# jingjing12110/X-GGM

Hardware: AMD Instinct MI355X
Metric: train samples/sec (36-obj VQA batch); one step = plain + GGM pass, each fwd+bwd+clip+BertAdam (higher is better)
Workload: dtype bf16; 1 GPU; 1xMI355X bf16: VQA-CP-v2-shaped synthetic batch=32/GPU, 36 objects x 2048, 20 tokens, A=2274, LXMERT 9/5/5 + GCNx2, full fwd+bwd+clip+BertAdam x2 passes (plain pass first, KL x 8), dropout on, delta=5 branch mix; global_batch=32, parallelism=dp1, order=vqa, world_size=1, zero1=False, hip_graph=True

## Files before the change

include/xggm.h:

```cpp
#ifndef XGGM_H
#define XGGM_H

#include <stddef.h>
#include <stdint.h>

#ifdef __cplusplus
extern "C" {
#endif

typedef struct ihipStream_t* xggm_stream_t;

#define XGGM_VERSION 100

#define XGGM_ACT_NONE 0
#define XGGM_ACT_GELU 1
#define XGGM_ACT_SIGMOID 2
#define XGGM_ACT_TANH 3
#define XGGM_ACT_GELU_GRAD 4

#define XGGM_AGG_PLAIN 0
#define XGGM_AGG_TRANSPOSE 1
#define XGGM_AGG_SYMMETRIZE 2

int xggm_version(void);
const char* xggm_last_error(void);
typedef struct xggm_prefetch { const void* ptr[4]; size_t bytes[4]; int n; } xggm_prefetch;

int xggm_gemm_f32(const void* A, const void* B, void* C, int M, int N, int K, int64_t a_rs, int64_t a_ks, int64_t b_ns,
                  int64_t b_ks, int64_t ldc, int batch, int64_t a_bs, int64_t b_bs, int64_t c_bs, const float* bias,
                  const void* residual, void* preact, const void* aux, float* colsum, int act, int c_f32, int accumulate,
                  float alpha, xggm_stream_t stream);
int xggm_gemm_bf16(const void* A, const void* B, void* C, int M, int N, int K, int64_t a_rs, int64_t a_ks, int64_t b_ns,
                   int64_t b_ks, int64_t ldc, int batch, int64_t a_bs, int64_t b_bs, int64_t c_bs, const float* bias,
                   const void* residual, void* preact, const void* aux, float* colsum, int act, int c_f32, int accumulate,
                   float alpha, xggm_stream_t stream);
typedef struct xggm_gemm_problem {
    const void* A;
    const void* B;
    void* C;
    int M, N, K;
    int64_t a_rs, a_ks, b_ns, b_ks, ldc;
    int batch;
    int64_t a_bs, b_bs, c_bs;
    const float* bias;
    const void* residual;
    void* preact;
    const void* aux;
    float* colsum;
    int act, c_f32, accumulate;
    float alpha;
    float* sqsum;
    const float* scale_a;
    const float* scale_b;
    void* c8;
    const float* c8_qscale;
    float* c8_amax;
    int amax_slots;
} xggm_gemm_problem;
int xggm_gemm_grouped_f32(const xggm_gemm_problem* probs, int n, int tile, xggm_stream_t stream);
int xggm_gemm_grouped_bf16(const xggm_gemm_problem* probs, int n, int tile, xggm_stream_t stream);
int xggm_gemm_fp8e4m3(const void* A, const void* B, void* C, int M, int N, int K, int64_t a_rs, int64_t b_ns, int64_t ldc,
                      const float* scale_a, const float* scale_b, const float* bias, const void* residual, void* preact,
                      int act, int c_f32, xggm_stream_t stream);
int xggm_gemm_grouped_fp8e4m3(const xggm_gemm_problem* probs, int n, int tile, xggm_stream_t stream);
int xggm_fp8_scale_update(float* amax, float* hist, float* qscale, float* dscale, int64_t* pos, int n, int hist_len,
                          float margin, int shrink, int bump, int amax_slots, xggm_stream_t stream);
int xggm_quantize_fp8e4m3_f32(const void* x, void* y, int64_t n, const float* qscale, float* amax, xggm_stream_t stream);
int xggm_quantize_fp8e4m3_bf16(const void* x, void* y, int64_t n, const float* qscale, float* amax, xggm_stream_t stream);
int xggm_gemm_set_group_tile(int v);
int xggm_gemm_set_generic(int on);
int xggm_gemm_set_tile(int variant);
int xggm_colsum_f32(const void* x, float* out, int M, int N, int64_t ld, float* ws, size_t ws_bytes,
                    xggm_stream_t stream);
int xggm_colsum_bf16(const void* x, float* out, int M, int N, int64_t ld, float* ws, size_t ws_bytes,
                     xggm_stream_t stream);
size_t xggm_colsum_workspace_bytes(int M, int N);

int xggm_attn_fwd_f32(const void* q, const void* k, const void* v, const float* mask, void* out, int B, int heads, int Sq,
                      int Sk, int head_dim, int64_t q_rs, int64_t k_rs, int64_t v_rs, int64_t o_rs, float scale, float p,
                      const uint64_t* rng, uint32_t sid, xggm_stream_t stream);
int xggm_attn_fwd_bf16(const void* q, const void* k, const void* v, const float* mask, void* out, int B, int heads, int Sq,
                       int Sk, int head_dim, int64_t q_rs, int64_t k_rs, int64_t v_rs, int64_t o_rs, float scale, float p,
                       const uint64_t* rng, uint32_t sid, xggm_stream_t stream);
int xggm_attn_bwd_f32(const void* q, const void* k, const void* v, const float* mask, const void* d_out, void* dq, void* dk,
                      void* dv, int B, int heads, int Sq, int Sk, int head_dim, int64_t q_rs, int64_t k_rs, int64_t v_rs,
                      int64_t o_rs, int64_t dq_rs, int64_t dk_rs, int64_t dv_rs, float scale, float p, const uint64_t* rng,
                      uint32_t sid, float* dbq, float* dbk, float* dbv, int64_t db_bs, xggm_stream_t stream);
int xggm_attn_bwd_bf16(const void* q, const void* k, const void* v, const float* mask, const void* d_out, void* dq,
                       void* dk, void* dv, int B, int heads, int Sq, int Sk, int head_dim, int64_t q_rs, int64_t k_rs,
                       int64_t v_rs, int64_t o_rs, int64_t dq_rs, int64_t dk_rs, int64_t dv_rs, float scale, float p,
                       const uint64_t* rng, uint32_t sid, float* dbq, float* dbk, float* dbv, int64_t db_bs,
                       xggm_stream_t stream);

typedef struct xggm_attn_problem {
    const void* q;
    const void* k;
    const void* v;
    const float* mask;
    void* out;
    int B, heads, Sq, Sk;
    int64_t q_rs, k_rs, v_rs, o_rs;
    float scale, p;
    uint32_t sid;
    const void* d_out;
    void* dq;
    void* dk;
    void* dv;
    int64_t dq_rs, dk_rs, dv_rs;
    float* dbq;
    float* dbk;
    float* dbv;
    int64_t db_bs;
    void* out8;
    const float* qscale;
    float* amax;
    int amax_slots;
} xggm_attn_problem;
int xggm_attn_fwd_grouped_f32(const xggm_attn_problem* probs, int n, int head_dim, const uint64_t* rng,
                              const xggm_prefetch* prefetch, xggm_stream_t stream);
int xggm_attn_fwd_grouped_bf16(const xggm_attn_problem* probs, int n, int head_dim, const uint64_t* rng,
                               const xggm_prefetch* prefetch, xggm_stream_t stream);
int xggm_attn_bwd_grouped_f32(const xggm_attn_problem* probs, int n, int head_dim, const uint64_t* rng,
                              const xggm_prefetch* prefetch, xggm_stream_t stream);
int xggm_attn_bwd_grouped_bf16(const xggm_attn_problem* probs, int n, int head_dim, const uint64_t* rng,
                               const xggm_prefetch* prefetch, xggm_stream_t stream);

int xggm_attn_set_scalar(int on);

int xggm_ln_fwd_f32(const void* in, const float* bias, const void* residual, const float* gamma, const float* beta,
                    void* out, void* z_out, float* stats, int M, int H, float eps, float p_pre, float p_post,
                    const uint64_t* rng, uint32_t sid_pre, uint32_t sid_post, int accumulate, float out_scale,
                    xggm_stream_t stream);
int xggm_ln_fwd_bf16(const void* in, const float* bias, const void* residual, const float* gamma, const float* beta,
                     void* out, void* z_out, float* stats, int M, int H, float eps, float p_pre, float p_post,
                     const uint64_t* rng, uint32_t sid_pre, uint32_t sid_post, int accumulate, float out_scale,
                     xggm_stream_t stream);
int xggm_ln_bwd_f32(const void* dy, const void* z, const float* stats, const float* gamma, void* d_in, void* d_res,
                    float* dgamma, float* dbeta, float* dbias, int M, int H, float p_pre, float p_post, const uint64_t* rng,
                    uint32_t sid_pre, uint32_t sid_post, float out_scale, int accumulate_dres, const void* gelu_aux,
                    float* ws, size_t ws_bytes, xggm_stream_t stream);
int xggm_ln_bwd_bf16(const void* dy, const void* z, const float* stats, const float* gamma, void* d_in, void* d_res,
                     float* dgamma, float* dbeta, float* dbias, int M, int H, float p_pre, float p_post,
                     const uint64_t* rng, uint32_t sid_pre, uint32_t sid_post, float out_scale, int accumulate_dres,
                     const void* gelu_aux, float* ws, size_t ws_bytes, xggm_stream_t stream);
typedef struct xggm_ln_fwd_problem {
    const void* in;
    const float* bias;
    const void* residual;
    const float* gamma;
    const float* beta;
    void* out;
    void* z_out;
    float* stats;
    int M;
    uint32_t sid_pre, sid_post;
    int in_slabs;
    void* out8;
    const float* qscale;
    float* amax;
    int amax_slots;
} xggm_ln_fwd_problem;
typedef struct xggm_ln_bwd_problem {
    const void* dy;
    const void* z;
    const float* stats;
    const float* gamma;
    void* d_in;
    void* d_res;
    float* dgamma;
    float* dbeta;
    float* dbias;
    const void* gelu_aux;
    float* ws;
    size_t ws_bytes;
    int M;
    uint32_t sid_pre, sid_post;
    int accumulate_dres;
} xggm_ln_bwd_problem;
int xggm_ln_fwd_grouped_f32(const xggm_ln_fwd_problem* probs, int n, int H, float eps, float p_pre, float p_post,
                            const uint64_t* rng, int accumulate, float out_scale, const xggm_prefetch* prefetch,
                            xggm_stream_t stream);
int xggm_ln_fwd_grouped_bf16(const xggm_ln_fwd_problem* probs, int n, int H, float eps, float p_pre, float p_post,
                             const uint64_t* rng, int accumulate, float out_scale, const xggm_prefetch* prefetch,
                             xggm_stream_t stream);
int xggm_ln_bwd_grouped_f32(const xggm_ln_bwd_problem* probs, int n, int H, float p_pre, float p_post,
                            const uint64_t* rng, float out_scale, const xggm_prefetch* prefetch, xggm_stream_t stream);
int xggm_ln_bwd_grouped_bf16(const xggm_ln_bwd_problem* probs, int n, int H, float p_pre, float p_post,
                             const uint64_t* rng, float out_scale, const xggm_prefetch* prefetch, xggm_stream_t stream);
typedef struct xggm_ln_sum_args {
    const void* in[4];
    const float* gamma[4];
    const float* beta[4];
    float* stats[4];
    uint32_t sid_post[4];
    void* out;
    int n, M, H;
    float eps, p_post;
    const uint64_t* rng;
} xggm_ln_sum_args;
int xggm_ln_sum_fwd_f32(const xggm_ln_sum_args* args, xggm_stream_t stream);
int xggm_ln_sum_fwd_bf16(const xggm_ln_sum_args* args, xggm_stream_t stream);
size_t xggm_ln_bwd_workspace_bytes(int M, int H);
size_t xggm_visn_embed_bwd_workspace_bytes(int M, int H);
typedef struct xggm_reduce_job {
    const float* ws;
    int nblk, K, H;
    float* target[3];
} xggm_reduce_job;
int xggm_partial_reduce_batch(const xggm_reduce_job* jobs, int n, xggm_stream_t stream);
int xggm_embed_fwd_f32(const int64_t* ids, const int64_t* seg, const void* word, const void* pos, const void* type,
                       const float* gamma, const float* beta, void* out, void* z_out, float* stats, int M, int Tlen, int H,
                       float eps, float p, const uint64_t* rng, uint32_t sid, void* out8, const float* qscale, float* amax,
                       int amax_slots, xggm_stream_t stream);
int xggm_embed_fwd_bf16(const int64_t* ids, const int64_t* seg, const void* word, const void* pos, const void* type,
                        const float* gamma, const float* beta, void* out, void* z_out, float* stats, int M, int Tlen, int H,
                        float eps, float p, const uint64_t* rng, uint32_t sid, void* out8, const float* qscale, float* amax,
                        int amax_slots, xggm_stream_t stream);
#define XGGM_SIDE_MAX 3
#define XGGM_SIDE_ADDITIVE_MASK 1
#define XGGM_SIDE_CAST_BF16 2
typedef struct xggm_side_jobs {
    int n;
    struct {
// ... 266 lines not shown
```

x-ggm_amd/csrc/gemm.hip:

```cpp
#include "common.h"
#include "xggm.h"

namespace {

typedef __attribute__((ext_vector_type(8))) short short8_t;
typedef __attribute__((ext_vector_type(4))) float float4_t;

struct GemmArgs {
    const void* A = nullptr;
    const void* B = nullptr;
    void* C = nullptr;
    int M = 0, N = 0, K = 0;
    int64_t a_rs = 0, a_ks = 0, b_ns = 0, b_ks = 0, ldc = 0;
    int64_t a_bs = 0, b_bs = 0, c_bs = 0;
    const float* bias = nullptr;
    const void* residual = nullptr;
    void* preact = nullptr;
    const void* aux = nullptr;
    float* colsum = nullptr;
    float* sqsum = nullptr;
    unsigned char* c8 = nullptr;
    const float* c8_qscale = nullptr;
    float* c8_amax = nullptr;
    int amax_slots = 1;
    const float* scale_a = nullptr;
    const float* scale_b = nullptr;
    int act = 0;
    int c_f32 = 0;
    int accumulate = 0;
    float alpha = 1.f;
    int a_mode = 0, b_mode = 0;
    int a_tail = 0, b_tail = 0;
    int a_rows = 0, b_rows = 0;
    int xcd_swizzle = 1;
    int batch = 1;
    int use_glds = 1;
    struct TileMap {
        int gx, gy, gxy;
        int xr, xc, rh, rw;
        int ncg, wb_last;
        unsigned m_rw, m_wbl, m_gxy;
    } tm = {};
#ifdef XGGM_STAMP
    long long* stamp = nullptr;
    int ablate = 0;
#endif
};

#ifdef XGGM_STAMP
long long* g_stamp = nullptr;
int g_ablate = 0;
#define ABLATE(g, bit) ((g).ablate & (bit))
#ifdef XGGM_KABLATE
#define KABLATE(g, bit) ((g).ablate & (bit))
#else
#define KABLATE(g, bit) false
#endif
#define STAMP(g, slot)                                                                                \
    do {                                                                                              \
        if ((g).stamp && threadIdx.x == 0)                                                            \
            (g).stamp[(int64_t)(blockIdx.x + gridDim.x * (blockIdx.y + gridDim.y * blockIdx.z)) * 8 + (slot)] = \
                __builtin_readcyclecounter();                                                         \
    } while (0)
#define SET_STAMP(g) ((g).stamp = g_stamp, (g).ablate = g_ablate)
#define STAMP_HW(g)                                                                                   \
    do {                                                                                              \
        if ((g).stamp && threadIdx.x == 0) {                                                          \
            unsigned hw, xcc;                                                                         \
            asm volatile("s_getreg_b32 %0, hwreg(HW_REG_HW_ID)" : "=s"(hw));                          \
            asm volatile("s_getreg_b32 %0, hwreg(HW_REG_XCC_ID)" : "=s"(xcc));                        \
            long long* q = (g).stamp + (int64_t)(blockIdx.x + gridDim.x * (blockIdx.y + gridDim.y * blockIdx.z)) * 8; \
            q[5] = hw;                                                                                \
            q[6] = xcc;                                                                               \
        }                                                                                             \
    } while (0)
#define XGGM_TRACE_BASE (8 * 8192)
__shared__ long long xg_trace[128];
#define TRACE(g, slot)                                                                                \
    do {                                                                                              \
        if (((g).ablate & 0x10000) && threadIdx.x == 0 && (slot) < 128) xg_trace[(slot)] = __builtin_readcyclecounter(); \
    } while (0)
#define TRACE_FLUSH(g)                                                                                \
    do {                                                                                              \
        if (((g).ablate & 0x10000) && threadIdx.x < 64) {                                                          \
            long long* q = (g).stamp + XGGM_TRACE_BASE +                                              \
                           (int64_t)(blockIdx.x + gridDim.x * (blockIdx.y + gridDim.y * blockIdx.z)) * 128; \
            q[threadIdx.x] = xg_trace[threadIdx.x];                                                   \
            q[threadIdx.x + 64] = xg_trace[threadIdx.x + 64];                                         \
        }                                                                                             \
    } while (0)
#else
#define TRACE(g, slot)
#define TRACE_FLUSH(g)
#define STAMP_HW(g)
#define ABLATE(g, bit) false
#define KABLATE(g, bit) false
#define STAMP(g, slot)
#define SET_STAMP(g)
#endif

template <typename T> struct Tile;
template <> struct Tile<bf16> {
    static constexpr int BK = 64;
    static constexpr int VEC = 8;
    static constexpr int LDK = BK + 8;
};
template <> struct Tile<float> {
    static constexpr int BK = 32;
    static constexpr int VEC = 4;
    static constexpr int LDK = BK + 4;
};

constexpr int BM = 64, BN = 64, NT = 256;
struct GemmHooks {
    bool force_generic = false;
    int tile_override = 0;
    int xcd_swizzle = 1;
    int glds_stages = 0;
    int single_grouped = 1;
    int no_8w = 0;
    int glds = 1;
    int group_tile = 0;
};
GemmHooks g_hooks;

template <typename T>
__device__ __forceinline__ void stage_tile(T* __restrict__ lds, const T* __restrict__ base, int64_t rs, int64_t ks, int r0,
                                           int k0, int R, int K, int mode, int tid) {
    constexpr int BK = Tile<T>::BK, VEC = Tile<T>::VEC, LDK = Tile<T>::LDK;
    typedef typename std::conditional<sizeof(T) == 2, short8_t, float4_t>::type vec_t;
    if (mode == 1) {
        constexpr int CPR = BK / VEC;
#pragma unroll
        for (int c = tid; c < 64 * CPR; c += NT) {
            const int row = c / CPR, kc = (c % CPR) * VEC;
            const int gr = r0 + row, gk = k0 + kc;
            vec_t v = {};
            if (gr < R && gk < K) v = *reinterpret_cast<const vec_t*>(base + (int64_t)gr * rs + gk);
            *reinterpret_cast<vec_t*>(lds + row * LDK + kc) = v;
        }
    } else if (mode == 2) {
        constexpr int CPL = 64 / VEC;
#pragma unroll
        for (int c = tid; c < BK * CPL; c += NT) {
            const int kl = c / CPL, rc = (c % CPL) * VEC;
            const int gr = r0 + rc, gk = k0 + kl;
            vec_t v = {};
            if (gr < R && gk < K) v = *reinterpret_cast<const vec_t*>(base + (int64_t)gk * ks + gr);
            const T* e = reinterpret_cast<const T*>(&v);
#pragma unroll
            for (int i = 0; i < VEC; ++i) lds[(rc + i) * LDK + kl] = e[i];
        }
    } else {
        for (int c = tid; c < 64 * BK; c += NT) {
            const int row = c / BK, kk = c % BK;
            const int gr = r0 + row, gk = k0 + kk;
            T v = from_f32<T>(0.0f);
            if (gr < R && gk < K) v = base[(int64_t)gr * rs + (int64_t)gk * ks];
            lds[row * LDK + kk] = v;
        }
    }
}

template <typename T> __device__ __forceinline__ float act_apply(int act, float v, float aux) {
    switch (act) {
        case XGGM_ACT_GELU: return gelu_f(v);
        case XGGM_ACT_SIGMOID: return sigmoid_f(v);
        case XGGM_ACT_TANH: return tanhf(v);
        case XGGM_ACT_GELU_GRAD: return v * gelu_grad_f(aux);
        default: return v;
    }
}

template <typename T>
__device__ __forceinline__ float epilogue_tile(const GemmArgs& g, const float4_t& acc, int row0, int col, int bz) {
    if (col >= g.N) return 0.f;
    const int64_t coff = (int64_t)bz * g.c_bs;
    const float bias = g.bias ? g.bias[col] : 0.0f;
    float csum = 0.f;
#pragma unroll
    for (int r = 0; r < 4; ++r) {
        const int row = row0 + r;
        if (row >= g.M) continue;
        const int64_t idx = coff + (int64_t)row * g.ldc + col;
        float v = g.alpha * acc[r] + bias;
        if (g.preact) reinterpret_cast<T*>(g.preact)[idx] = from_f32<T>(v);
        float aux = 0.0f;
        if (g.act == XGGM_ACT_GELU_GRAD) aux = to_f32(reinterpret_cast<const T*>(g.aux)[idx]);
        if (g.act != XGGM_ACT_NONE) {
            if (g.preact) v = round_to<T>(v);
            v = act_apply<T>(g.act, v, aux);
        }
        if (g.residual) v += to_f32(reinterpret_cast<const T*>(g.residual)[idx]);
        if (g.c_f32) {
            float* c = reinterpret_cast<float*>(g.C) + idx;
            *c = g.accumulate ? (*c + v) : v;
        } else {
            T* c = reinterpret_cast<T*>(g.C) + idx;
            *c = from_f32<T>(g.accumulate ? (to_f32(*c) + v) : v);
        }
        csum += v;
    }
    return csum;
}

template <typename T> __global__ __launch_bounds__(NT) void gemm_kernel(GemmArgs g) {
    constexpr int BK = Tile<T>::BK, LDK = Tile<T>::LDK;
    __shared__ __attribute__((aligned(16))) T As[BM * LDK];
    __shared__ __attribute__((aligned(16))) T Bs[BN * LDK];

    const int tid = threadIdx.x, lane = tid & 63, wid = tid >> 6;
    const int wm = (wid >> 1) * 32, wn = (wid & 1) * 32;
    const int m0 = blockIdx.y * BM, n0 = blockIdx.x * BN, bz = blockIdx.z;
    const T* A = reinterpret_cast<const T*>(g.A) + (int64_t)bz * g.a_bs;
    const T* B = reinterpret_cast<const T*>(g.B) + (int64_t)bz * g.b_bs;

    float4_t acc[2][2];
#pragma unroll
    for (int i = 0; i < 2; ++i)
#pragma unroll
        for (int j = 0; j < 2; ++j) acc[i][j] = (float4_t){0.f, 0.f, 0.f, 0.f};

    const int fr = lane & 15, fq = lane >> 4;
    for (int k0 = 0; k0 < g.K; k0 += BK) {
        stage_tile<T>(As, A, g.a_rs, g.a_ks, m0, k0, g.M, g.K, g.a_mode, tid);
        stage_tile<T>(Bs, B, g.b_ns, g.b_ks, n0, k0, g.N, g.K, g.b_mode, tid);
        __syncthreads();
        if constexpr (sizeof(T) == 2) {
#pragma unroll
            for (int ks = 0; ks < BK; ks += 32) {
                short8_t a[2], b[2];
#pragma unroll
                for (int i = 0; i < 2; ++i) {
                    a[i] = *reinterpret_cast<const short8_t*>(As + (wm + i * 16 + fr) * LDK + ks + fq * 8);
                    b[i] = *reinterpret_cast<const short8_t*>(Bs + (wn + i * 16 + fr) * LDK + ks + fq * 8);
                }
#pragma unroll
                for (int i = 0; i < 2; ++i)
#pragma unroll
                    for (int j = 0; j < 2; ++j)
                        acc[i][j] = __builtin_amdgcn_mfma_f32_16x16x32_bf16(
                            __builtin_bit_cast(__attribute__((ext_vector_type(8))) __bf16, a[i]),
                            __builtin_bit_cast(__attribute__((ext_vector_type(8))) __bf16, b[j]), acc[i][j], 0, 0, 0);
            }
        } else {
#pragma unroll
            for (int ks = 0; ks < BK; ks += 4) {
                float a[2], b[2];
#pragma unroll
                for (int i = 0; i < 2; ++i) {
                    a[i] = As[(wm + i * 16 + fr) * LDK + ks + fq];
                    b[i] = Bs[(wn + i * 16 + fr) * LDK + ks + fq];
                }
#pragma unroll
                for (int i = 0; i < 2; ++i)
#pragma unroll
                    for (int j = 0; j < 2; ++j)
                        acc[i][j] = __builtin_amdgcn_mfma_f32_16x16x4f32(a[i], b[j], acc[i][j], 0, 0, 0);
            }
        }
        __syncthreads();
    }

#pragma unroll
    for (int j = 0; j < 2; ++j) {
        float cs = 0.f;
#pragma unroll
        for (int i = 0; i < 2; ++i) cs += epilogue_tile<T>(g, acc[i][j], m0 + wm + i * 16 + fq * 4, n0 + wn + j * 16 + fr, bz);
        if (g.colsum) {
            cs += __shfl_xor(cs, 16, 64);
            cs += __shfl_xor(cs, 32, 64);
            const int col = n0 + wn + j * 16 + fr, slot = (m0 + wm) >> 5;
            if (fq == 0 && col < g.N && m0 + wm < g.M)
                g.colsum[((int64_t)bz * ((g.M + 31) >> 5) + slot) * g.N + col] = cs;
        }
// ... 1054 lines not shown
        else gemm_kloop_glds<BM, BN, true, false, false, W, NS>(g, tile_m, tile_n, bz, fsm, acc);                    \
    } else {                                                                                                         \
        if (g.b_mode == 1) gemm_kloop_glds<BM, BN, false, true, false, W, NS>(g, tile_m, tile_n, bz, fsm, acc);      \
        else gemm_kloop_glds<BM, BN, false, false, false, W, NS>(g, tile_m, tile_n, bz, fsm, acc);                   \
    }
        if (ga.stages == 2) { XGGM_GLDS_FORMS(2) }
        else if (ga.stages == 3) { XGGM_GLDS_FORMS(3) }
        else { XGGM_GLDS_FORMS(4) }
#undef XGGM_GLDS_FORMS
    } else if (g.a_mode == 1) {
        if (g.b_mode == 1) gemm_kloop<BM, BN, true, true, DK, false, W>(g, tile_m, tile_n, bz, fsm, acc);
        else gemm_kloop<BM, BN, true, false, DK, false, W>(g, tile_m, tile_n, bz, fsm, acc);
    } else {
        if (g.b_mode == 1) gemm_kloop<BM, BN, false, true, DK, false, W>(g, tile_m, tile_n, bz, fsm, acc);
        else gemm_kloop<BM, BN, false, false, 2, false, W>(g, tile_m, tile_n, bz, fsm, acc);
    }
    gemm_finish<BM, BN, W>(g, tile_m, tile_n, bz, fsm, acc);
}

template <int BM, int BN, int W = 4> int launch_grouped_tile(GroupArgs& ga, const GemmHooks& h, hipStream_t stream) {
    int total;
    if (int e = layout_group(ga, BM, BN, &total)) return e;
    ga.stages = h.glds_stages ? h.glds_stages : (W == 4 && 2 * 3 * sizeof(bf16) * (BM + BN) * 64 > 160 * 1024) ? 2 : 3;
    while (ga.stages > 2 && ga.stages * sizeof(bf16) * (BM + BN) * 64 > 160 * 1024) --ga.stages;
    size_t lds = 0;
    for (int i = 0; i < ga.nprob; ++i) {
        const size_t a = ga.p[i].a_mode == 1 ? OpLds<BM, true>::ELEMS : OpLds<BM, false>::ELEMS;
        const size_t b = ga.p[i].b_mode == 1 ? OpLds<BN, true>::ELEMS : OpLds<BN, false>::ELEMS;
        lds = std::max(lds, glds_ok<false>(ga.p[i]) ? ga.stages * sizeof(bf16) * (BM + BN) * 64 : 2 * sizeof(bf16) * (a + b));
    }
    if (int e = xggm_reserve_lds(reinterpret_cast<const void*>(&gemm_grouped_kernel<BM, BN, W>), lds, "xggm_gemm_grouped")) return e;
    hipLaunchKernelGGL((gemm_grouped_kernel<BM, BN, W>), dim3(total), dim3(64 * W), lds, stream, ga);
    return xggm_check_launch("xggm_gemm_grouped");
}

constexpr int ROLE_NS = 3;
template <int BM, int BN> constexpr int role_min_waves() { return BM * BN >= 128 * 128 ? 2 : 4; }

template <int BM, int BN>
__global__ __launch_bounds__(512, (role_min_waves<BM, BN>())) void gemm_grouped_role_kernel(GroupArgs ga) {
    extern __shared__ __attribute__((aligned(16))) bf16 fsm[];
    const int b = blockIdx.x;
    int i = 0, t0 = 0, t1 = ga.tile_start[1];
#pragma unroll
    for (int k = 1; k < MAX_GROUP; ++k)
        if (k < ga.nprob && b >= ga.tile_start[k]) { i = k; t0 = ga.tile_start[k]; t1 = ga.tile_start[k + 1]; }
    const GemmArgs g = ga.p[i];
    int tile_m, tile_n, bz;
    tile_from_map(g, b - t0, t1 - t0, tile_m, tile_n, bz);
    STAMP(g, 0);
    STAMP_HW(g);
    const int wid = __builtin_amdgcn_readfirstlane((int)(threadIdx.x >> 6));
    if (wid >= 4) {
        if (g.a_mode == 1) {
            if (g.b_mode == 1) gemm_role_load<BM, BN, true, true, ROLE_NS>(g, tile_m, tile_n, bz, fsm, wid - 4);
            else gemm_role_load<BM, BN, true, false, ROLE_NS>(g, tile_m, tile_n, bz, fsm, wid - 4);
        } else {
            if (g.b_mode == 1) gemm_role_load<BM, BN, false, true, ROLE_NS>(g, tile_m, tile_n, bz, fsm, wid - 4);
            else gemm_role_load<BM, BN, false, false, ROLE_NS>(g, tile_m, tile_n, bz, fsm, wid - 4);
        }
        return;
    }
    float4_t acc[BM / 32][BN / 32];
    if (g.a_mode == 1) {
        if (g.b_mode == 1) gemm_role_compute<BM, BN, true, true, ROLE_NS>(g, fsm, acc);
        else gemm_role_compute<BM, BN, true, false, ROLE_NS>(g, fsm, acc);
    } else {
        if (g.b_mode == 1) gemm_role_compute<BM, BN, false, true, ROLE_NS>(g, fsm, acc);
        else gemm_role_compute<BM, BN, false, false, ROLE_NS>(g, fsm, acc);
    }
    gemm_finish<BM, BN, 4>(g, tile_m, tile_n, bz, fsm, acc);
}

template <int BM, int BN> int launch_grouped_role(GroupArgs& ga, hipStream_t stream) {
    int total;
    if (int e = layout_group(ga, BM, BN, &total)) return e;
    ga.stages = ROLE_NS;
    constexpr size_t lds = std::max(ROLE_NS * sizeof(bf16) * (BM + BN) * 64, sizeof(float) * (BM / 2) * (BN + 4));
    if (int e = xggm_reserve_lds(reinterpret_cast<const void*>(&gemm_grouped_role_kernel<BM, BN>), lds, "xggm_gemm_grouped(role)"))
        return e;
    hipLaunchKernelGGL((gemm_grouped_role_kernel<BM, BN>), dim3(total), dim3(512), lds, stream, ga);
    return xggm_check_launch("xggm_gemm_grouped(role)");
}

template <int BM, int BN, int W = 4>
__global__ __launch_bounds__(64 * W, (W == 8 ? 2 : min_waves<BM, BN>())) void gemm_grouped_fp8_kernel(GroupArgs ga) {
    extern __shared__ __attribute__((aligned(16))) bf16 fsm[];
    const int b = blockIdx.x;
    int i = 0, t0 = 0, t1 = ga.tile_start[1];
#pragma unroll
    for (int k = 1; k < MAX_GROUP; ++k)
        if (k < ga.nprob && b >= ga.tile_start[k]) { i = k; t0 = ga.tile_start[k]; t1 = ga.tile_start[k + 1]; }
    GemmArgs g = ga.p[i];
    int tile_m, tile_n, bz;
    tile_from_map(g, b - t0, t1 - t0, tile_m, tile_n, bz);
    constexpr int DK = (BM * BN <= 64 * 64) ? 4 : 2;
    float4_t acc[BM / (8 * W)][BN / 32];
    const float deq = (g.scale_a ? *g.scale_a : 1.f) * (g.scale_b ? *g.scale_b : 1.f);
    if (glds_ok<true>(g)) {
        if (ga.stages == 3) gemm_kloop_glds<BM, BN, true, true, true, W, 3>(g, tile_m, tile_n, bz, fsm, acc);
        else gemm_kloop_glds<BM, BN, true, true, true, W, 2>(g, tile_m, tile_n, bz, fsm, acc);
    } else {
        gemm_kloop<BM, BN, true, true, DK, true, W>(g, tile_m, tile_n, bz, fsm, acc);
    }
    g.alpha *= deq;
    gemm_finish<BM, BN, W>(g, tile_m, tile_n, bz, fsm, acc);
}

template <int BM, int BN, int W = 4> int launch_grouped_fp8_tile(GroupArgs& ga, const GemmHooks& h, hipStream_t stream) {
    int total;
    if (int e = layout_group(ga, BM, BN, &total)) return e;
    ga.stages = h.glds_stages ? std::min(h.glds_stages, 3) : (BM * BN == 128 * 128 && W == 4) ? 2 : 3;
    bool glds = true;
    for (int i = 0; i < ga.nprob; ++i) glds = glds && glds_ok<true>(ga.p[i]);
    const size_t lds = std::max((glds ? ga.stages : 2) * sizeof(bf16) * (OpLds<BM, true>::ELEMS + OpLds<BN, true>::ELEMS),
                                sizeof(float) * (BM / 2) * (BN + 4));
    if (int e = xggm_reserve_lds(reinterpret_cast<const void*>(&gemm_grouped_fp8_kernel<BM, BN, W>), lds, "xggm_gemm_grouped_fp8e4m3"))
        return e;
    hipLaunchKernelGGL((gemm_grouped_fp8_kernel<BM, BN, W>), dim3(total), dim3(64 * W), lds, stream, ga);
    return xggm_check_launch("xggm_gemm_grouped_fp8e4m3");
}

template <int BM, int BN, int D> int launch_fast_tile(const GemmArgs& g, int batch, hipStream_t stream) {
    dim3 grid(ceil_div(g.N, BN), ceil_div(g.M, BM), batch);
    const bool ak = g.a_mode == 1, bk = g.b_mode == 1;
#define XGGM_FAST(AKv, BKv)                                                                                           \
    do {                                                                                                              \
        constexpr size_t lds = 2 * sizeof(bf16) * (OpLds<BM, AKv>::ELEMS + OpLds<BN, BKv>::ELEMS);                   \
        if (int e = xggm_reserve_lds(reinterpret_cast<const void*>(&gemm_fast_kernel<BM, BN, AKv, BKv, D>), lds,      \
                                     "xggm_gemm(fast)")) return e;                                                    \
        hipLaunchKernelGGL((gemm_fast_kernel<BM, BN, AKv, BKv, D>), grid, dim3(NT), lds, stream, g);                  \
    } while (0)
    if (ak && bk) XGGM_FAST(true, true);
    else if (ak && !bk) XGGM_FAST(true, false);
    else if (!ak && bk) XGGM_FAST(false, true);
    else XGGM_FAST(false, false);
#undef XGGM_FAST
    return xggm_check_launch("xggm_gemm(fast)");
}

inline int launch_fast(const GemmArgs& g, int batch, int v, hipStream_t stream) {
    if (v == 0) v = (g.a_mode == 2 && g.b_mode == 2) ? 1 : 2;
    switch (v) {
        case 6: return launch_fast_tile<64, 64, 1>(g, batch, stream);
        case 7: return launch_fast_tile<128, 64, 1>(g, batch, stream);
        case 8: return launch_fast_tile<128, 128, 1>(g, batch, stream);
        case 1: return launch_fast_tile<64, 64, 2>(g, batch, stream);
        case 2: return launch_fast_tile<64, 64, 4>(g, batch, stream);
        case 3: return launch_fast_tile<128, 64, 2>(g, batch, stream);
        default: return launch_fast_tile<128, 128, 2>(g, batch, stream);
    }
}

template <typename T> int pick_mode(const void* base, int64_t rs, int64_t ks, int64_t bs, int R, int K, int* tail, int* rows) {
    constexpr int VEC = Tile<T>::VEC;
    *tail = 0;
    *rows = R;
    const bool base_ok = (reinterpret_cast<uintptr_t>(base) % 16 == 0) && (bs % VEC == 0);
    if (ks == 1 && base_ok && rs % VEC == 0) {
        if (K % VEC == 0) return 1;
        if (sizeof(T) == 2 && K % 2 == 0 && rs >= (K + VEC - 1) / VEC * VEC) {
            *tail = 1;
            return 1;
        }
    }
    if (rs == 1 && base_ok && ks % VEC == 0) {
        if (R % VEC == 0) return 2;
        if (sizeof(T) == 2 && ks >= (R + VEC - 1) / VEC * VEC) {
            *rows = (R + VEC - 1) / VEC * VEC;
            return 2;
        }
    }
    return 0;
}

GemmArgs from_problem(const xggm_gemm_problem& p, const GemmHooks& h) {
    GemmArgs g;
    g.A = p.A; g.B = p.B; g.C = p.C; g.M = p.M; g.N = p.N; g.K = p.K;
    g.a_rs = p.a_rs; g.a_ks = p.a_ks; g.b_ns = p.b_ns; g.b_ks = p.b_ks; g.ldc = p.ldc;
    g.a_bs = p.a_bs; g.b_bs = p.b_bs; g.c_bs = p.c_bs;
    g.bias = p.bias; g.residual = p.residual; g.preact = p.preact; g.aux = p.aux; g.colsum = p.colsum; g.sqsum = p.sqsum;
    g.c8 = reinterpret_cast<unsigned char*>(p.c8); g.c8_qscale = p.c8_qscale; g.c8_amax = p.c8_amax;
    g.amax_slots = p.amax_slots > 1 ? p.amax_slots : 1;
    g.scale_a = p.scale_a; g.scale_b = p.scale_b;
    g.act = p.act; g.c_f32 = p.c_f32; g.accumulate = p.accumulate; g.alpha = p.alpha;
    g.xcd_swizzle = h.xcd_swizzle; g.batch = p.batch; g.use_glds = h.glds; SET_STAMP(g);
    return g;
}

template <typename T> int launch(GemmArgs g, int batch, const GemmHooks& h, hipStream_t stream) {
    XGGM_REQUIRE(g.M > 0 && g.N > 0 && g.K > 0 && batch > 0, "xggm_gemm: empty problem M=%d N=%d K=%d batch=%d", g.M, g.N,
                 g.K, batch);
    XGGM_REQUIRE(g.A && g.B && g.C, "xggm_gemm: null operand");
    XGGM_REQUIRE(g.act >= 0 && g.act <= XGGM_ACT_GELU_GRAD, "xggm_gemm: bad activation %d", g.act);
    XGGM_REQUIRE(g.act != XGGM_ACT_GELU_GRAD || g.aux, "xggm_gemm: GELU_GRAD needs aux");
    XGGM_REQUIRE(g.ldc >= g.N, "xggm_gemm: ldc %lld < N %d", (long long)g.ldc, g.N);
    XGGM_REQUIRE(!g.sqsum || g.c_f32, "xggm_gemm: sqsum is defined for fp32 outputs");
    g.a_mode = pick_mode<T>(g.A, g.a_rs, g.a_ks, g.a_bs, g.M, g.K, &g.a_tail, &g.a_rows);
    g.b_mode = pick_mode<T>(g.B, g.b_ns, g.b_ks, g.b_bs, g.N, g.K, &g.b_tail, &g.b_rows);
    dim3 grid(ceil_div(g.N, BN), ceil_div(g.M, BM), batch);
    XGGM_REQUIRE(grid.y <= 65535 && grid.z <= 65535, "xggm_gemm: grid too large");
    if constexpr (sizeof(T) == 2) {
        if (g.a_mode != 0 && g.b_mode != 0 && !h.force_generic) return launch_fast(g, batch, h.tile_override, stream);
    }
    XGGM_REQUIRE(!g.sqsum, "xggm_gemm: sqsum needs the tuned bf16 kernels (8-aligned operands); this problem runs on the "
                           "generic kernel");
    if (g.a_tail || g.a_rows != g.M) g.a_mode = 0;
    if (g.b_tail || g.b_rows != g.N) g.b_mode = 0;
    hipLaunchKernelGGL(gemm_kernel<T>, grid, dim3(NT), 0, stream, g);
    return xggm_check_launch("xggm_gemm");
}

}

#define XGGM_GEMM_IMPL(NAME, T)                                                                                        \
    extern "C" int NAME(const void* A, const void* B, void* C, int M, int N, int K, int64_t a_rs, int64_t a_ks,       \
                        int64_t b_ns, int64_t b_ks, int64_t ldc, int batch, int64_t a_bs, int64_t b_bs, int64_t c_bs, \
                        const float* bias, const void* residual, void* preact, const void* aux, float* colsum,       \
                        int act, int c_f32, int accumulate, float alpha, hipStream_t stream) {                        \
        const GemmHooks h = g_hooks;                                                                                   \
        xggm_gemm_problem p = {};                                                                                      \
        p.A = A; p.B = B; p.C = C; p.M = M; p.N = N; p.K = K;                                                          \
        p.a_rs = a_rs; p.a_ks = a_ks; p.b_ns = b_ns; p.b_ks = b_ks; p.ldc = ldc;                                       \
        p.batch = batch; p.a_bs = a_bs; p.b_bs = b_bs; p.c_bs = c_bs;                                                  \
        p.bias = bias; p.residual = residual; p.preact = preact; p.aux = aux; p.colsum = colsum;                      \
        p.act = act; p.c_f32 = c_f32; p.accumulate = accumulate; p.alpha = alpha;                                     \
        return launch<T>(from_problem(p, h), batch, h, stream);                                                        \
    }

XGGM_GEMM_IMPL(xggm_gemm_f32, float)
XGGM_GEMM_IMPL(xggm_gemm_bf16, bf16)

extern "C" int xggm_gemm_fp8e4m3(const void* A, const void* B, void* C, int M, int N, int K, int64_t a_rs, int64_t b_ns,
                                 int64_t ldc, const float* scale_a, const float* scale_b, const float* bias,
                                 const void* residual, void* preact, int act, int c_f32, hipStream_t stream) {
    XGGM_REQUIRE(M > 0 && N > 0 && K > 0, "xggm_gemm_fp8e4m3: empty problem M=%d N=%d K=%d", M, N, K);
    XGGM_REQUIRE(A && B && C, "xggm_gemm_fp8e4m3: null operand");
    XGGM_REQUIRE(K % 16 == 0 && a_rs % 16 == 0 && b_ns % 16 == 0 && a_rs >= K && b_ns >= K,
                 "xggm_gemm_fp8e4m3: K and the row strides must be multiples of 16 (K=%d, strides %lld, %lld)", K,
                 (long long)a_rs, (long long)b_ns);
    XGGM_REQUIRE(reinterpret_cast<uintptr_t>(A) % 16 == 0 && reinterpret_cast<uintptr_t>(B) % 16 == 0,
                 "xggm_gemm_fp8e4m3: operands must be 16-byte aligned");
    XGGM_REQUIRE(act >= 0 && act < XGGM_ACT_GELU_GRAD, "xggm_gemm_fp8e4m3: bad activation %d", act);
    XGGM_REQUIRE(ldc >= N, "xggm_gemm_fp8e4m3: ldc %lld < N %d", (long long)ldc, N);
    XGGM_REQUIRE((int64_t)(M - 1) * a_rs + K < OOB_OFFSET && (int64_t)(N - 1) * b_ns + K < OOB_OFFSET,
                 "xggm_gemm_fp8e4m3: operand larger than 2 GiB");
    const GemmHooks h = g_hooks;
    xggm_gemm_problem p = {};
    p.A = A; p.B = B; p.C = C; p.M = M; p.N = N; p.K = K;
    p.a_rs = a_rs; p.a_ks = 1; p.b_ns = b_ns; p.b_ks = 1; p.ldc = ldc; p.batch = 1;
    p.bias = bias; p.residual = residual; p.preact = preact; p.act = act; p.c_f32 = c_f32; p.alpha = 1.0f;
    GemmArgs g = from_problem(p, h);
    g.a_mode = g.b_mode = 1; g.a_rows = M; g.b_rows = N;
    switch (h.tile_override) {
        case 3: return launch_fp8_tile<128, 64, 2>(g, scale_a, scale_b, stream);
        case 5: return launch_fp8_tile<128, 128, 2>(g, scale_a, scale_b, stream);
        case 1: return launch_fp8_tile<64, 64, 2>(g, scale_a, scale_b, stream);
        default: return launch_fp8_tile<64, 64, 4>(g, scale_a, scale_b, stream);
    }
}

extern "C" int xggm_gemm_set_generic(int on) {
    g_hooks.force_generic = on != 0;
    return XGGM_OK;
}

extern "C" int xggm_gemm_set_tile(int variant) {
    g_hooks.tile_override = variant & 0xff;
    g_hooks.xcd_swizzle = (variant & 0x100) ? 0 : 1;
    g_hooks.glds = (variant & 0x400) ? 0 : 1;
    g_hooks.no_8w = (variant & 0x4000) ? 1 : 0;
    g_hooks.single_grouped = (variant & 0x8000) ? 0 : 1;
    g_hooks.glds_stages = (variant & 0x800) ? 2 : (variant & 0x1000) ? 3 : (variant & 0x2000) ? 4 : 0;
    return XGGM_OK;
}

namespace {
int pick_group_tile(const GroupArgs& ga, int n, int kt, int tile) {
    struct TileModel { int bm, bn; float a, b, s, f, k; };
    struct TileModels { TileModel m[3]; };
    static const TileModels tuned = [] {
        TileModels t{{{64, 64, 3.3f, 1.2f, 0.19f, 5.0f, 0.28f},
                      {128, 64, 4.2f, 2.0f, 0.37f, 5.6f, 0.56f},
                      {128, 128, 2.3f, 6.1f, 0.71f, 8.4f, 0.75f}}};
        if (const char* e = getenv("XGGM_TILE_MODEL")) {
            float q[15];
            if (sscanf(e, "%f,%f,%f,%f,%f;%f,%f,%f,%f,%f;%f,%f,%f,%f,%f", q, q + 1, q + 2, q + 3, q + 4, q + 5, q + 6, q + 7,
                       q + 8, q + 9, q + 10, q + 11, q + 12, q + 13, q + 14) == 15)
                for (int c = 0; c < 3; ++c) {
                    t.m[c].a = q[5 * c]; t.m[c].b = q[5 * c + 1]; t.m[c].s = q[5 * c + 2];
                    t.m[c].f = q[5 * c + 3]; t.m[c].k = q[5 * c + 4];
                }
        }
        return t;
    }();
    int v = tile;
    if (v == 0) {
        float best = 0.f;
        for (int c = 0; c < 3; ++c) {
            const TileModel& tm = tuned.m[c];
            double tiles = 0, work = 0;
            int nkmax = 0;
            for (int i = 0; i < n; ++i) {
                const double t = (double)ceil_div(ga.p[i].M, tm.bm) * ceil_div(ga.p[i].N, tm.bn) * ga.p[i].batch;
                const int nk = ceil_div(ga.p[i].K, kt);
                tiles += t;
                work += t * nk;
                nkmax = std::max(nkmax, nk);
            }
            const float r = std::max(1.0, tiles / 256.0);
            const float est = std::max(tm.a + tm.b * r + tm.s * (float)(work / 256.0), tm.f + tm.k * nkmax);
            if (v == 0 || est < best) {
                best = est;
                v = c + 1;
            }
        }
    }
    return v;
}

inline bool group_tile_ok(int tile) { return (tile >= 0 && tile <= 4) || (tile >= 7 && tile <= 9); }

template <typename T> int grouped(const xggm_gemm_problem* probs, int n, int tile, const GemmHooks h, hipStream_t stream) {
    XGGM_REQUIRE(probs && n > 0, "xggm_gemm_grouped: no problems");
    XGGM_REQUIRE(group_tile_ok(tile), "xggm_gemm_grouped: tile %d (0: the library chooses; 1-4, 7-9: see xggm.h)", tile);
    const int pin = tile ? tile : h.group_tile;
    bool fast = sizeof(T) == 2 && !h.force_generic && n <= MAX_GROUP;
    GroupArgs ga;
    ga.nprob = n;
    for (int i = 0; i < n && fast; ++i) {
        GemmArgs g = from_problem(probs[i], h);
        if (!(g.M > 0 && g.N > 0 && g.K > 0 && g.batch > 0 && g.A && g.B && g.C)) fast = false;
        g.a_mode = pick_mode<T>(g.A, g.a_rs, g.a_ks, g.a_bs, g.M, g.K, &g.a_tail, &g.a_rows);
        g.b_mode = pick_mode<T>(g.B, g.b_ns, g.b_ks, g.b_bs, g.N, g.K, &g.b_tail, &g.b_rows);
        if (g.a_mode == 0 || g.b_mode == 0) fast = false;
        ga.p[i] = g;
    }
    for (int i = 1; i < n && fast; ++i)
        for (int j = i; j > 0 && ga.p[j].K > ga.p[j - 1].K; --j) std::swap(ga.p[j], ga.p[j - 1]);
    if (!fast || (n == 1 && !(h.single_grouped && glds_ok<false>(ga.p[0])))) {
        for (int i = 0; i < n; ++i)
            if (int e = launch<T>(from_problem(probs[i], h), probs[i].batch, h, stream)) return e;
        return XGGM_OK;
    }
    int v = pick_group_tile(ga, n, 64, pin);
    if (pin == 0 && sizeof(T) == 2) {
        int64_t t128 = 0;
        bool kmaj = true;
        int nkmin = 1 << 30;
        for (int i = 0; i < n; ++i) {
            t128 += (int64_t)ceil_div(ga.p[i].M, 128) * ceil_div(ga.p[i].N, 128) * ga.p[i].batch;
            kmaj = kmaj && ga.p[i].a_mode == 1 && ga.p[i].b_mode == 1;
            nkmin = std::min(nkmin, ceil_div(ga.p[i].K, 64));
        }
        if (kmaj && t128 > 200 && t128 <= 256 && nkmin >= 12 && !h.no_8w) v = 4;
        else if (t128 >= 448) v = 3;
    }
#ifdef XGGM_BIG_TILES
    if (v == 5) return launch_grouped_tile<128, 256, 8>(ga, h, stream);
    if (v == 6) return launch_grouped_tile<256, 128, 8>(ga, h, stream);
#endif
    if (v >= 7 && v <= 9) {
        bool ok = true;
        for (int i = 0; i < n; ++i) ok = ok && glds_ok<false>(ga.p[i]);
        if (ok)
            return v == 7 ? launch_grouped_role<128, 128>(ga, stream)
                          : v == 8 ? launch_grouped_role<128, 64>(ga, stream) : launch_grouped_role<64, 64>(ga, stream);
        v = v == 7 ? 3 : v == 8 ? 2 : 1;
    }
    if (v == 4) return launch_grouped_tile<128, 128, 8>(ga, h, stream);
    if (v == 3) return launch_grouped_tile<128, 128>(ga, h, stream);
    if (v == 2) return launch_grouped_tile<128, 64>(ga, h, stream);
    return launch_grouped_tile<64, 64>(ga, h, stream);
}
}

extern "C" int xggm_gemm_grouped_fp8e4m3(const xggm_gemm_problem* probs, int n, int tile, hipStream_t stream) {
    XGGM_REQUIRE(probs && n > 0 && n <= MAX_GROUP, "xggm_gemm_grouped_fp8e4m3: 1..%d problems per launch (n = %d)", MAX_GROUP, n);
    XGGM_REQUIRE(group_tile_ok(tile), "xggm_gemm_grouped_fp8e4m3: tile %d (0: the library chooses; 1-4, 7-9: see xggm.h)", tile);
    const GemmHooks h = g_hooks;
    const int pin = tile ? tile : h.group_tile;
    GroupArgs ga;
    ga.nprob = n;
    for (int i = 0; i < n; ++i) {
        GemmArgs g = from_problem(probs[i], h);
        XGGM_REQUIRE(g.M > 0 && g.N > 0 && g.K > 0 && g.batch > 0 && g.A && g.B && g.C,
                     "xggm_gemm_grouped_fp8e4m3: empty problem or null operand (%d)", i);
        XGGM_REQUIRE(g.a_ks == 1 && g.b_ks == 1, "xggm_gemm_grouped_fp8e4m3: e4m3 operands are k-contiguous");
        XGGM_REQUIRE(g.K % 16 == 0 && g.a_rs % 16 == 0 && g.b_ns % 16 == 0 && g.a_rs >= g.K && g.b_ns >= g.K &&
                         g.a_bs % 16 == 0 && g.b_bs % 16 == 0,
                     "xggm_gemm_grouped_fp8e4m3: K, row and batch strides must be multiples of 16 (K = %d)", g.K);
        XGGM_REQUIRE(reinterpret_cast<uintptr_t>(g.A) % 16 == 0 && reinterpret_cast<uintptr_t>(g.B) % 16 == 0,
                     "xggm_gemm_grouped_fp8e4m3: operands must be 16-byte aligned");
        XGGM_REQUIRE(g.act >= 0 && g.act < XGGM_ACT_GELU_GRAD && !g.aux && !g.colsum && !g.sqsum && !g.accumulate,
                     "xggm_gemm_grouped_fp8e4m3: forward epilogues only");
        XGGM_REQUIRE(g.ldc >= g.N, "xggm_gemm_grouped_fp8e4m3: ldc %lld < N %d", (long long)g.ldc, g.N);
        XGGM_REQUIRE(!g.c8 || (g.ldc % 8 == 0 && g.N % 8 == 0 && reinterpret_cast<uintptr_t>(g.c8) % 8 == 0 && !g.c_f32),
                     "xggm_gemm_grouped_fp8e4m3: the e4m3 copy needs an 8-aligned bf16 output");
        XGGM_REQUIRE((int64_t)(g.M - 1) * g.a_rs + (int64_t)(g.batch - 1) * g.a_bs + g.K < OOB_OFFSET &&
                         (int64_t)(g.N - 1) * g.b_ns + (int64_t)(g.batch - 1) * g.b_bs + g.K < OOB_OFFSET,
                     "xggm_gemm_grouped_fp8e4m3: operand larger than 2 GiB");
        g.a_mode = g.b_mode = 1;
        g.a_rows = g.M;
        g.b_rows = g.N;
        ga.p[i] = g;
    }
    for (int i = 1; i < n; ++i)
        for (int j = i; j > 0 && ga.p[j].K > ga.p[j - 1].K; --j) std::swap(ga.p[j], ga.p[j - 1]);
    int v = pick_group_tile(ga, n, 128, pin);
    if (pin == 0) {
        static const bool use8 = getenv("XGGM_FP8_8W") && atoi(getenv("XGGM_FP8_8W")) == 1;
        int64_t t128 = 0;
        for (int i = 0; i < n; ++i) t128 += (int64_t)ceil_div(ga.p[i].M, 128) * ceil_div(ga.p[i].N, 128) * ga.p[i].batch;
        if (use8 && t128 > 200 && t128 <= 256 && !h.no_8w) v = 4;
    }
    if (v == 4) return launch_grouped_fp8_tile<128, 128, 8>(ga, h, stream);
    if (v == 3) return launch_grouped_fp8_tile<128, 128>(ga, h, stream);
    if (v == 2) return launch_grouped_fp8_tile<128, 64>(ga, h, stream);
    return launch_grouped_fp8_tile<64, 64>(ga, h, stream);
}
extern "C" int xggm_gemm_grouped_bf16(const xggm_gemm_problem* probs, int n, int tile, hipStream_t stream) {
    return grouped<bf16>(probs, n, tile, g_hooks, stream);
}
extern "C" int xggm_gemm_grouped_f32(const xggm_gemm_problem* probs, int n, int tile, hipStream_t stream) {
    return grouped<float>(probs, n, tile, g_hooks, stream);
}
#ifdef XGGM_STAMP
extern "C" int xggm_gemm_occupancy(int tile, int lds_bytes, int* out) {
    int n = -1;
    hipError_t e;
    if (tile == 3) e = hipOccupancyMaxActiveBlocksPerMultiprocessor(&n, gemm_grouped_kernel<128, 128>, NT, lds_bytes);
    else if (tile == 2) e = hipOccupancyMaxActiveBlocksPerMultiprocessor(&n, gemm_grouped_kernel<128, 64>, NT, lds_bytes);
    else e = hipOccupancyMaxActiveBlocksPerMultiprocessor(&n, gemm_grouped_kernel<64, 64>, NT, lds_bytes);
    hipDeviceProp_t pr;
    (void)hipGetDeviceProperties(&pr, 0);
    out[0] = n;
    out[1] = (int)pr.maxSharedMemoryPerMultiProcessor;
    out[2] = (int)pr.sharedMemPerBlock;
    out[3] = pr.regsPerMultiprocessor;
    out[4] = pr.regsPerBlock;
    out[5] = (int)e;
    return XGGM_OK;
}
extern "C" int xggm_gemm_set_ablate(int bits) {
    g_ablate = bits;
    return XGGM_OK;
}
extern "C" int xggm_gemm_set_stamp(long long* buf) {
    g_stamp = buf;
    return XGGM_OK;
}
#endif
extern "C" int xggm_gemm_set_group_tile(int v) {
    g_hooks.group_tile = v;
    return XGGM_OK;
}
```

Measured before the change: 2984 samples/s.

## Add skinny GEMM kernels for small-M and small-K bf16 problems

Adds a dedicated skinny GEMM path with two shapes. When M is at most 32 it splits K across eight waves and reduces the partial sums through LDS. When K is at most 32 with f32 output, typical of batch-32 weight-gradient and classifier shapes, it uses a single-slab MFMA kernel. Both single and grouped launches route to it by default, and it can be turned off with the XGGM_SKINNY environment variable. This aims to avoid wasting 64- and 128-wide tiles and serial K loops on these shapes, at the cost of an LDS reduction and more code paths to keep correct.

```diff
diff --git a/include/xggm.h b/include/xggm.h
--- a/include/xggm.h
+++ b/include/xggm.h
@@ -69,6 +69,7 @@
 int xggm_quantize_fp8e4m3_bf16(const void* x, void* y, int64_t n, const float* qscale, float* amax, xggm_stream_t stream);
 int xggm_gemm_set_group_tile(int v);
 int xggm_gemm_set_generic(int on);
+int xggm_gemm_set_skinny(int on);
 int xggm_gemm_set_tile(int variant);
 int xggm_colsum_f32(const void* x, float* out, int M, int N, int64_t ld, float* ws, size_t ws_bytes,
                     xggm_stream_t stream);
diff --git a/x-ggm_amd/csrc/gemm.hip b/x-ggm_amd/csrc/gemm.hip
--- a/x-ggm_amd/csrc/gemm.hip
+++ b/x-ggm_amd/csrc/gemm.hip
@@ -121,6 +121,7 @@
     int no_8w = 0;
     int glds = 1;
     int group_tile = 0;
+    int skinny = !(getenv("XGGM_SKINNY") && atoi(getenv("XGGM_SKINNY")) == 0);
 };
 GemmHooks g_hooks;
 
@@ -1481,6 +1482,244 @@
     }
 }
 
+constexpr int SK_W = 8, SK_NT = 64 * SK_W;
+constexpr int SK_SLAB_M = 128, SK_SLAB_N = 64, SK_SLAB_LD = 40;
+enum : int { SK_NONE = 0, SK_ROWS_K = 1, SK_ROWS_N = 2, SK_SLAB = 4 };
+struct SkinnyArgs {
+    GemmArgs p[MAX_GROUP];
+    int start[MAX_GROUP + 1];
+    int kind[MAX_GROUP];
+    int nprob;
+};
+
+__device__ __forceinline__ short8_t skinny_k8(const bf16* row, int k, int K) {
+    short8_t v = {0, 0, 0, 0, 0, 0, 0, 0};
+    if (row && k < K) {
+        v = *reinterpret_cast<const short8_t*>(row + k);
+        if (k + 8 > K) {
+#pragma unroll
+            for (int j = 1; j < 8; ++j)
+                if (k + j >= K) v[j] = 0;
+        }
+    }
+    return v;
+}
+
+__device__ __forceinline__ void skinny_store(const GemmArgs& g, float acc, int row, int col) {
+    const int64_t idx = (int64_t)row * g.ldc + col;
+    float v = g.alpha * acc + (g.bias ? g.bias[col] : 0.f);
+    if (g.preact) {
+        const bf16 t = __float2bfloat16(v);
+        reinterpret_cast<bf16*>(g.preact)[idx] = t;
+        v = __bfloat162float(t);
+    }
+    if (g.act == XGGM_ACT_GELU) v = gelu_f(v);
+    else if (g.act != XGGM_ACT_NONE) v = act_apply<bf16>(g.act, v, 0.f);
+    if (g.residual) v += __bfloat162float(reinterpret_cast<const bf16*>(g.residual)[idx]);
+    if (g.c_f32) {
+        float* c = reinterpret_cast<float*>(g.C) + idx;
+        *c = g.accumulate ? (*c + v) : v;
+    } else {
+        bf16* c = reinterpret_cast<bf16*>(g.C) + idx;
+        *c = __float2bfloat16(g.accumulate ? (__bfloat162float(*c) + v) : v);
+    }
+}
+
+template <bool BK> __device__ __forceinline__ void skinny_rows(const GemmArgs& g, int blk, float* red) {
+    constexpr int CT = BK ? 2 : 4, CB = 16 * CT, E = CT * 4;
+    const int tid = threadIdx.x, lane = tid & 63, wid = tid >> 6, fr = lane & 15, fq = lane >> 4;
+    const int n0 = blk * CB;
+    const bf16* A = reinterpret_cast<const bf16*>(g.A);
+    const bf16* B = reinterpret_cast<const bf16*>(g.B);
+    const bf16* arow[2] = {fr < g.M ? A + (int64_t)fr * g.a_rs : nullptr, fr + 16 < g.M ? A + (int64_t)(fr + 16) * g.a_rs : nullptr};
+    float4_t acc[2][CT];
+#pragma unroll
+    for (int i = 0; i < 2; ++i)
+#pragma unroll
+        for (int j = 0; j < CT; ++j) acc[i][j] = (float4_t){0.f, 0.f, 0.f, 0.f};
+    const int nch = (g.K + 31) >> 5;
+    for (int c = wid; c < nch; c += 2 * SK_W) {
+        short8_t a[2][2], b[2][CT];
+#pragma unroll
+        for (int u = 0; u < 2; ++u) {
+            const int k = (c + u * SK_W) * 32 + fq * 8;
+            a[u][0] = skinny_k8(arow[0], k, g.K);
+            a[u][1] = skinny_k8(arow[1], k, g.K);
+            if constexpr (BK) {
+#pragma unroll
+                for (int j = 0; j < CT; ++j) {
+                    const int n = n0 + j * 16 + fr;
+                    b[u][j] = skinny_k8(n < g.N ? B + (int64_t)n * g.b_ns : nullptr, k, g.K);
+                }
+            } else {
+                const int col = n0 + 4 * fr;
+                short4_t v[8];
+#pragma unroll
+                for (int i = 0; i < 8; ++i) {
+                    v[i] = (short4_t){0, 0, 0, 0};
+                    if (k + i < g.K && col < g.b_rows) v[i] = *reinterpret_cast<const short4_t*>(B + (int64_t)(k + i) * g.b_ks + col);
+                }
+#pragma unroll
+                for (int j = 0; j < CT; ++j)
+#pragma unroll
+                    for (int i = 0; i < 8; ++i) b[u][j][i] = v[i][j];
+            }
+        }
+#pragma unroll
+        for (int u = 0; u < 2; ++u)
+#pragma unroll
+            for (int i = 0; i < 2; ++i)
+#pragma unroll
+                for (int j = 0; j < CT; ++j)
+                    acc[i][j] = __builtin_amdgcn_mfma_f32_16x16x32_bf16(__builtin_bit_cast(bf16x8_t, a[u][i]),
+                                                                        __builtin_bit_cast(bf16x8_t, b[u][j]), acc[i][j], 0, 0, 0);
+    }
+    const int mtiles = g.M > 16 ? 2 : 1;
+    for (int mt = 0; mt < mtiles; ++mt) {
+        if (mt) __syncthreads();
+#pragma unroll
+        for (int j = 0; j < CT; ++j)
+#pragma unroll
+            for (int r = 0; r < 4; ++r) red[(wid * E + j * 4 + r) * 64 + lane] = mt ? acc[1][j][r] : acc[0][j][r];
+        __syncthreads();
+        const int rows = min(16, g.M - mt * 16);
+        for (int o = tid; o < rows * CB; o += SK_NT) {
+            const int lr = o / CB, col = o % CB, n = n0 + col;
+            if (n >= g.N) continue;
+            const int j = BK ? col >> 4 : col & 3, cl = BK ? col & 15 : col >> 2;
+            const int at = (j * 4 + (lr & 3)) * 64 + (lr >> 2) * 16 + cl;
+            float s = red[at];
+#pragma unroll
+            for (int w = 1; w < SK_W; ++w) s += red[w * E * 64 + at];
+            skinny_store(g, s, mt * 16 + lr, n);
+        }
+    }
+}
+
+__device__ __forceinline__ void skinny_slab(const GemmArgs& g, int blk, bf16* lds) {
+    const int tid = threadIdx.x, lane = tid & 63, wid = tid >> 6, fr = lane & 15, fq = lane >> 4;
+    const int gx = (g.N + SK_SLAB_N - 1) / SK_SLAB_N;
+    const int m0 = (blk / gx) * SK_SLAB_M, n0 = (blk % gx) * SK_SLAB_N;
+    const int wm = (wid >> 1) * 32, wn = (wid & 1) * 32;
+    const bf16* A = reinterpret_cast<const bf16*>(g.A);
+    const bf16* B = reinterpret_cast<const bf16*>(g.B);
+    float* C = reinterpret_cast<float*>(g.C);
+    bf16* As = lds;
+    bf16* Bs = lds + SK_SLAB_M * SK_SLAB_LD;
+    const bool vec = (g.ldc % 4 == 0) && (reinterpret_cast<uintptr_t>(g.C) % 16 == 0);
+    float4_t prev[2][2];
+#pragma unroll
+    for (int i = 0; i < 2; ++i)
+#pragma unroll
+        for (int j = 0; j < 2; ++j) {
+            const int m = m0 + wm + i * 16 + fr, n = n0 + wn + j * 16 + fq * 4;
+            prev[i][j] = (float4_t){0.f, 0.f, 0.f, 0.f};
+            if (g.accumulate && vec && m < g.M && n + 3 < g.N) prev[i][j] = *reinterpret_cast<const float4_t*>(C + (int64_t)m * g.ldc + n);
+        }
+    {
+        const int kl = tid >> 4, rc = (tid & 15) * 8;
+        short8_t v = {0, 0, 0, 0, 0, 0, 0, 0};
+        if (kl < g.K && m0 + rc < g.a_rows) v = *reinterpret_cast<const short8_t*>(A + (int64_t)kl * g.a_ks + m0 + rc);
+#pragma unroll
+        for (int i = 0; i < 8; ++i) reinterpret_cast<short*>(As)[(rc + i) * SK_SLAB_LD + kl] = v[i];
+    }
+    if (tid < 256) {
+        const int kl = tid >> 3, rc = (tid & 7) * 8;
+        short8_t v = {0, 0, 0, 0, 0, 0, 0, 0};
+        if (kl < g.K && n0 + rc < g.b_rows) v = *reinterpret_cast<const short8_t*>(B + (int64_t)kl * g.b_ks + n0 + rc);
+#pragma unroll
+        for (int i = 0; i < 8; ++i) reinterpret_cast<short*>(Bs)[(rc + i) * SK_SLAB_LD + kl] = v[i];
+    }
+    __syncthreads();
+    short8_t a[2], b[2];
+#pragma unroll
+    for (int i = 0; i < 2; ++i) {
+        a[i] = *reinterpret_cast<const short8_t*>(As + (wm + i * 16 + fr) * SK_SLAB_LD + fq * 8);
+        b[i] = *reinterpret_cast<const short8_t*>(Bs + (wn + i * 16 + fr) * SK_SLAB_LD + fq * 8);
+    }
+#pragma unroll
+    for (int i = 0; i < 2; ++i)
+#pragma unroll
+        for (int j = 0; j < 2; ++j) {
+            const float4_t d = __builtin_amdgcn_mfma_f32_16x16x32_bf16(__builtin_bit_cast(bf16x8_t, b[j]), __builtin_bit_cast(bf16x8_t, a[i]),
+                                                                       (float4_t){0.f, 0.f, 0.f, 0.f}, 0, 0, 0);
+            const int m = m0 + wm + i * 16 + fr, n = n0 + wn + j * 16 + fq * 4;
+            if (m >= g.M || n >= g.N) continue;
+            float* c = C + (int64_t)m * g.ldc + n;
+            if (vec && n + 3 < g.N) {
+                *reinterpret_cast<float4_t*>(c) = prev[i][j] + g.alpha * d;
+            } else {
+#pragma unroll
+                for (int r = 0; r < 4; ++r)
+                    if (n + r < g.N) c[r] = g.accumulate ? (c[r] + g.alpha * d[r]) : g.alpha * d[r];
+            }
+        }
+}
+
+template <int KINDS> __global__ __launch_bounds__(SK_NT) void gemm_skinny_kernel(SkinnyArgs sa) {
+    extern __shared__ __attribute__((aligned(16))) float sk_lds[];
+    const int b = blockIdx.x;
+    int i = 0;
+#pragma unroll
+    for (int k = 1; k < MAX_GROUP; ++k)
+        if (k < sa.nprob && b >= sa.start[k]) i = k;
+    const GemmArgs g = sa.p[i];
+    const int kind = sa.kind[i], blk = b - sa.start[i];
+    if ((KINDS & SK_ROWS_K) && kind == SK_ROWS_K) skinny_rows<true>(g, blk, sk_lds);
+    else if ((KINDS & SK_ROWS_N) && kind == SK_ROWS_N) skinny_rows<false>(g, blk, sk_lds);
+    else if ((KINDS & SK_SLAB) && kind == SK_SLAB) skinny_slab(g, blk, reinterpret_cast<bf16*>(sk_lds));
+}
+
+inline int skinny_kind(const GemmArgs& g, const GemmHooks& h) {
+    if (!h.skinny || h.force_generic || g.batch != 1) return SK_NONE;
+    if (!(g.M > 0 && g.N > 0 && g.K > 0 && g.A && g.B && g.C) || g.ldc < g.N) return SK_NONE;
+    if (g.aux || g.colsum || g.sqsum || g.c8 || g.scale_a || g.scale_b) return SK_NONE;
+    if (g.M <= 32 && g.a_mode == 1 && g.b_mode != 0 && g.act >= XGGM_ACT_NONE && g.act <= XGGM_ACT_TANH)
+        return g.b_mode == 1 ? SK_ROWS_K : SK_ROWS_N;
+    if (g.K <= 32 && g.a_mode == 2 && g.b_mode == 2 && g.c_f32 && g.act == XGGM_ACT_NONE && !g.bias && !g.residual && !g.preact)
+        return SK_SLAB;
+    return SK_NONE;
+}
+
+template <int KINDS> int launch_skinny_kinds(const SkinnyArgs& sa, int total, size_t lds, hipStream_t stream) {
+    hipLaunchKernelGGL((gemm_skinny_kernel<KINDS>), dim3(total), dim3(SK_NT), lds, stream, sa);
+    return xggm_check_launch("xggm_gemm(skinny)");
+}
+
+int launch_skinny(const GemmArgs* p, const int* kinds, int n, hipStream_t stream) {
+    SkinnyArgs sa;
+    sa.nprob = n;
+    int64_t t = 0;
+    int mask = 0;
+    size_t lds = 0;
+    for (int i = 0; i < n; ++i) {
+        sa.p[i] = p[i];
+        sa.kind[i] = kinds[i];
+        sa.start[i] = (int)t;
+        mask |= kinds[i];
+        if (kinds[i] == SK_SLAB) {
+            t += (int64_t)ceil_div(p[i].M, SK_SLAB_M) * ceil_div(p[i].N, SK_SLAB_N);
+            lds = std::max(lds, sizeof(bf16) * (SK_SLAB_M + SK_SLAB_N) * SK_SLAB_LD);
+        } else {
+            const int ct = kinds[i] == SK_ROWS_K ? 2 : 4;
+            t += ceil_div(p[i].N, 16 * ct);
+            lds = std::max(lds, sizeof(float) * SK_W * ct * 4 * 64);
+        }
+        XGGM_REQUIRE(t <= INT32_MAX, "xggm_gemm(skinny): more than 2^31 - 1 workgroups in one launch");
+    }
+    for (int i = n; i < MAX_GROUP; ++i) sa.kind[i] = SK_NONE;
+    for (int i = n; i <= MAX_GROUP; ++i) sa.start[i] = (int)t;
+    switch (mask) {
+        case 1: return launch_skinny_kinds<1>(sa, (int)t, lds, stream);
+        case 2: return launch_skinny_kinds<2>(sa, (int)t, lds, stream);
+        case 3: return launch_skinny_kinds<3>(sa, (int)t, lds, stream);
+        case 4: return launch_skinny_kinds<4>(sa, (int)t, lds, stream);
+        case 5: return launch_skinny_kinds<5>(sa, (int)t, lds, stream);
+        case 6: return launch_skinny_kinds<6>(sa, (int)t, lds, stream);
+        default: return launch_skinny_kinds<7>(sa, (int)t, lds, stream);
+    }
+}
+
 template <typename T> int pick_mode(const void* base, int64_t rs, int64_t ks, int64_t bs, int R, int K, int* tail, int* rows) {
     constexpr int VEC = Tile<T>::VEC;
     *tail = 0;
@@ -1530,6 +1769,7 @@
     dim3 grid(ceil_div(g.N, BN), ceil_div(g.M, BM), batch);
     XGGM_REQUIRE(grid.y <= 65535 && grid.z <= 65535, "xggm_gemm: grid too large");
     if constexpr (sizeof(T) == 2) {
+        if (const int kind = skinny_kind(g, h)) return launch_skinny(&g, &kind, 1, stream);
         if (g.a_mode != 0 && g.b_mode != 0 && !h.force_generic) return launch_fast(g, batch, h.tile_override, stream);
     }
     XGGM_REQUIRE(!g.sqsum, "xggm_gemm: sqsum needs the tuned bf16 kernels (8-aligned operands); this problem runs on the "
@@ -1594,6 +1834,11 @@
     return XGGM_OK;
 }
 
+extern "C" int xggm_gemm_set_skinny(int on) {
+    g_hooks.skinny = on != 0;
+    return XGGM_OK;
+}
+
 extern "C" int xggm_gemm_set_tile(int variant) {
     g_hooks.tile_override = variant & 0xff;
     g_hooks.xcd_swizzle = (variant & 0x100) ? 0 : 1;
@@ -1664,6 +1909,12 @@
         g.b_mode = pick_mode<T>(g.B, g.b_ns, g.b_ks, g.b_bs, g.N, g.K, &g.b_tail, &g.b_rows);
         if (g.a_mode == 0 || g.b_mode == 0) fast = false;
         ga.p[i] = g;
+    }
+    if constexpr (sizeof(T) == 2) {
+        int kinds[MAX_GROUP];
+        bool all = fast;
+        for (int i = 0; i < n && all; ++i) all = (kinds[i] = skinny_kind(ga.p[i], h)) != SK_NONE;
+        if (all) return launch_skinny(ga.p, kinds, n, stream);
     }
     for (int i = 1; i < n && fast; ++i)
         for (int j = i; j > 0 && ga.p[j].K > ga.p[j - 1].K; --j) std::swap(ga.p[j], ga.p[j - 1]);
```

Result: no change. 2958 samples/s (-0.9%).
